# lzc452/SSL-VIT-VIDEO-ANALYTICS

Hardware: AMD Instinct MI355X
Metric: clips/sec (8x3x224x224) MAE ViT-Tiny pretrain, 1/2/4/8 GPU + recon-loss parity (higher is better)
Workload: dtype bf16; 1 GPU; BASELINE config 2: TinyViT-21M-variant MAE (stem+stages 1-3) + 4x384 decoder, T=8, 224x224, mask 0.75, bf16 autocast; model=tiny_vit_21m_variant + TinyVideoMAE, global_batch=256, per_gpu_batch=256, frames=8, image_size=224, parallelism=dp1

## Files before the change

include/sm_api.h:

```cpp
#ifndef SM_API_H
#define SM_API_H
#include <stdint.h>
#include <hip/hip_runtime_api.h>

#ifdef __cplusplus
extern "C" {
#endif

int64_t sm_gemm_workspace_bytes(int ab_dtype, int M, int N, int K);
int sm_gemm(int ab_dtype, int c_dtype, int a_layout, int b_layout, int M, int N, int K,
            const void* A, int64_t lda, const void* B, int64_t ldb, void* C, int64_t ldc,
            const float* bias, float alpha, float beta, int epi, void* aux, const void* R,
            float drop_p, uint64_t seed, const float* row_scale, int64_t rows_per_group,
            void* workspace, int64_t ws_bytes, hipStream_t stream);
int sm_gemm_persistent(int mode);
int sm_gemm_tuning(int key, int set, int value, int* prev);
int64_t sm_linear_dw_bias_workspace_bytes(int rows, int nout, int nin);
int sm_linear_dw_bias(int rows, int nout, int nin, const void* dy, const void* x, float* dW, float* db,
                      int accumulate, void* ws, int64_t ws_bytes, hipStream_t stream);
int sm_linear_dx_gelu(int M, int N, int K, const void* dy, const void* w, const void* pre, void* dx, void* h,
                      float drop_p, uint64_t seed, hipStream_t stream);
int sm_linear_dw_bias_gelu(int rows, int nout, int nin, const void* dy, const void* pre, float drop_p,
                           uint64_t seed, float* dW, float* db, int accumulate, void* ws, int64_t ws_bytes,
                           hipStream_t stream);
// ... 137 lines not shown
int64_t sm_se_workspace_bytes(int F, int HW, int C);
int sm_se_fwd(int dtype, const void* x, const float* act_mean, const float* act_rstd, const float* act_w,
              const float* act_b, int act_gelu, int F, int HW, int C, int R, const float* w1, const float* w2,
              float* pooled, float* z1, float* s, void* y, void* ws, int64_t ws_bytes, hipStream_t st);
int sm_se_bwd(int dtype, const void* dy, const void* x, const float* act_mean, const float* act_rstd,
              const float* act_w, const float* act_b, int act_gelu, int F, int HW, int C, int R,
              const float* w1, const float* w2, const float* s, const float* z1, float* dz2, float* dz1,
              void* dx, void* ws, int64_t ws_bytes, hipStream_t st);
int sm_se_scale(int dtype, const void* x, const float* act_mean, const float* act_rstd, const float* act_w,
                const float* act_b, int act_gelu, const float* s, void* y, int F, int HW, int C, hipStream_t st);
int64_t sm_se_bn_bwd_workspace_bytes(int F, int HW, int C);
int sm_se_bn_bwd(int dtype, const void* dy, const void* x, const float* bn_mean, const float* bn_rstd,
                 const float* bn_w, const float* bn_b, int bn_gelu, int F, int HW, int C, int R, const float* w1,
                 const float* w2, const float* s, const float* z1, float* dz2, float* dz1, void* dx, float* dw,
                 float* db, void* ws, int64_t ws_bytes, hipStream_t st);

int sm_tube_mask(const float* noise, int B, int T, int L, int n_mask, uint8_t* mask, int32_t* idx,
                 hipStream_t st);
int sm_pos_blend_fwd(int y_dtype, int x_dtype, const void* y, const float* tpos, const float* spos,
                     const float* tok, const uint8_t* mask, void* x, int B, int T, int L, int D,
                     hipStream_t st);
int sm_pos_blend_bwd(int g_dtype, int y_dtype, const void* dx, const uint8_t* mask, void* dy,
                     float* dtpos, float* dspos, float* dtok, float* ws, int B, int T, int L, int D,
                     hipStream_t st);
int64_t sm_loss_workspace_bytes(int B, int T, int L);
int sm_mae_loss_fwd(int pred_dtype, const void* pred, const float* clip, int64_t sB, int64_t sC,
                    int64_t sT, int64_t sH, int64_t sW, const uint8_t* mask, int B, int T, int H, int W,
                    int norm_pix, float* loss, float* denom, void* ws, int64_t ws_bytes, hipStream_t st);
int sm_mae_loss_bwd(int pred_dtype, const void* pred, const float* clip, int64_t sB, int64_t sC,
                    int64_t sT, int64_t sH, int64_t sW, const uint8_t* mask, int B, int T, int H, int W,
// ... 58 lines not shown
```

ssl-vit-video-analytics_amd/csrc/common.h:

```cpp
#pragma once
#include <hip/hip_runtime.h>
#include <stdint.h>

#define SM_DEV __device__ __forceinline__

typedef __attribute__((ext_vector_type(8))) __bf16 bf16x8;
typedef __attribute__((ext_vector_type(4))) __bf16 bf16x4;
typedef __attribute__((ext_vector_type(16))) float f32x16;
typedef __attribute__((ext_vector_type(4))) float f32x4;
typedef __attribute__((ext_vector_type(4))) short s16x4;

enum SmDtype { SM_F32 = 0, SM_BF16 = 1 };

template <typename T> SM_DEV float to_f(T x);
template <> SM_DEV float to_f<float>(float x) { return x; }
template <> SM_DEV float to_f<__bf16>(__bf16 x) { return (float)x; }
template <typename T> SM_DEV T from_f(float x);
template <> SM_DEV float from_f<float>(float x) { return x; }
template <> SM_DEV __bf16 from_f<__bf16>(float x) { return (__bf16)x; }

SM_DEV void load8(const float* p, float* v) {
  float4 a = *(const float4*)p, b = *(const float4*)(p + 4);
  v[0] = a.x; v[1] = a.y; v[2] = a.z; v[3] = a.w; v[4] = b.x; v[5] = b.y; v[6] = b.z; v[7] = b.w;
}
// ... 216 lines not shown
  __syncthreads();
  if (g == 0 && c < ncols) {
    double t = 0.0;
#pragma unroll
    for (int k = 0; k < 8; ++k) t += red[k][cl];
    if (outd) outd[c] = t;
    if (outf) outf[c] = accumulate ? outf[c] + (float)t : (float)t;
  }
}

static inline void colred(const float* part, int nb, int ncols, double* outd, float* outf, int accumulate, hipStream_t st) {
  hipLaunchKernelGGL(colred_kernel, dim3((ncols + 31) / 32), dim3(256), 0, st, part, nb, ncols, outd, outf,
                     accumulate);
}

#define SM_CHECK_LAUNCH() \
  do { hipError_t e__ = hipGetLastError(); if (e__ != hipSuccess) return (int)e__; } while (0)
```

ssl-vit-video-analytics_amd/csrc/conv.hip:

```cpp
#include <algorithm>

#include "common.h"
#include "sm_api.h"

namespace {

inline int ew_blocks(int64_t n) {
  int64_t b = (n + 255) / 256;
  if (b > 16384) b = 16384;
  return b < 1 ? 1 : (int)b;
}

struct ClipView {
  const float* p;
  int B, T, H, W;
  int64_t sB, sC, sT, sH, sW;
};

template <typename TO>
__global__ void stem_im2col_kernel(ClipView v, int Ho, int Wo, int stride, TO* col ) {
  const int64_t P = (int64_t)v.B * v.T * Ho * Wo;
  for (int64_t i = blockIdx.x * (int64_t)blockDim.x + threadIdx.x; i < P; i += (int64_t)gridDim.x * blockDim.x) {
    const int xo = (int)(i % Wo);
    const int64_t r = i / Wo;
// ... 2010 lines not shown
  double* sums = (double*)(((uintptr_t)(coef + 2 * C) + 7) & ~(uintptr_t)7);
  ChanAffine act{bn_mean, bn_rstd, bn_w, bn_b, bn_gelu};
  DISPATCH1(dtype, hipLaunchKernelGGL(se_bn_reduce_kernel<T>, dim3(ns, F), dim3(256), 0, st, (const T*)dy,
                                      (const T*)x, act, HW, C, part, part2));
  hipLaunchKernelGGL(se_fc_bwd_kernel, dim3(F), dim3(256), (C + R) * 4, st, part, ns, s, z1, w1, w2, C, R, dz2, dz1,
                     dpool);
  hipLaunchKernelGGL(se_bn_combine_kernel, dim3(F), dim3(256), 0, st, part2, ns, HW, C, s, dpool, comb);
  colred(comb, F, 2 * C, sums, nullptr, 0, st);
  hipLaunchKernelGGL(se_bn_finalize_kernel, dim3((C + 127) / 128), dim3(128), 0, st, sums, (int64_t)F * HW, C, dw,
                     db, coef);
  DISPATCH1(dtype, hipLaunchKernelGGL(se_bn_dx_kernel<T>, dim3(ns, F), dim3(256), 0, st, (const T*)dy, (const T*)x,
                                      act, s, dpool, coef, (T*)dx, HW, C));
  SM_CHECK_LAUNCH();
  return 0;
}
```

ssl-vit-video-analytics_amd/csrc/gemm.hip:

```cpp
#include "common.h"
#include "sm_api.h"
#include <stdlib.h>

namespace {

struct GemmArgs {
  int M, N, K;
  int k_begin, k_chunk;
  const void* A; int64_t lda;
  const void* B; int64_t ldb;
  void* C; int64_t ldc;
  const float* bias;
  float alpha, beta;
  int epi;
  void* aux;
  const void* R;
  float drop_p;
  uint64_t seed;
  const float* row_scale;
  int64_t rows_per_group;
  float* partial;
  float* colsum;
  int cH, cW, cC, cflip;
  float xb_p;
  uint64_t xb_seed;
  ChanAffine xb_act;
  const float* xb_gate;
  int xb_hw;
  float* stat_part;
  int ctrans;
  void* aux_out;
  const void* A2;
  int64_t lda2;
  int k1;
};

template <typename TC>
SM_DEV void epilogue_store(const GemmArgs& g, int64_t row, int col, float acc, int zs) {
  if (g.partial) {
    g.partial[(int64_t)zs * g.M * g.N + row * g.N + col] = acc;
    return;
  }
  float v = g.alpha * acc;
  if (g.bias) v += g.bias[col];
  TC* C = (TC*)g.C;
  const int64_t idx = g.ctrans ? (int64_t)col * g.ldc + row : row * g.ldc + col;
  if (g.epi & 2) v = (float)(__bf16)v;
  if (g.epi & 4) v *= gelu_grad(to_f<TC>(((const TC*)g.aux)[idx]));
  if (g.epi & 1) {
// ... 1201 lines not shown
    const int wrow = (m0 + wm) >> 6;
    const int sc = n0 + wn + 8 * l;
    const auto prs = __builtin_amdgcn_make_buffer_rsrc((void*)(g.stat_part + (int64_t)wrow * 2 * g.N), (short)0,
                                                       2 * g.N * 4, 0x00020000);
    const bool ok = l < 8 && m0 + wm < g.M && sc < g.N;
    const uint32_t o = ok ? (uint32_t)sc * 4u : BUF_OOB;
    const uint32_t o2 = ok ? (uint32_t)(g.N + sc) * 4u : BUF_OOB;
    bstore128(make_uint4(__float_as_uint(st1[0]), __float_as_uint(st1[1]), __float_as_uint(st1[2]), __float_as_uint(st1[3])), prs, o);
    bstore128(make_uint4(__float_as_uint(st1[4]), __float_as_uint(st1[5]), __float_as_uint(st1[6]), __float_as_uint(st1[7])), prs, o + 16);
    bstore128(make_uint4(__float_as_uint(st2[0]), __float_as_uint(st2[1]), __float_as_uint(st2[2]), __float_as_uint(st2[3])), prs, o2);
    bstore128(make_uint4(__float_as_uint(st2[4]), __float_as_uint(st2[5]), __float_as_uint(st2[6]), __float_as_uint(st2[7])), prs, o2 + 16);
  }
  asm volatile("s_waitcnt lgkmcnt(0)" ::: "memory");
}

template <bool BK, int IMP>
__global__ __launch_bounds__(512, 4) void gemm_bf16_pp(GemmArgs g) {
  static_assert(IMP == 0 || IMP == 8 || IMP == 9 || IMP == 11 || IMP == 12 || IMP == 13,
                "persistent form: plain, statistics, GELU backward + activation, BatchNorm-input (+ statistics) "
                "or GELU + pre epilogue");
  constexpr bool STATS = IMP == 8 || IMP == 11;
  constexpr bool XA = IMP == 11 || IMP == 12;
  __shared__ float xtab[XA ? 2 * XB_MAXK : 4];
  constexpr int BMV = 256, BNV = 128, NT = 512;
  constexpr int CHA = TileLoader<BMV, NT, true>::CH, CHB = TileLoader<BNV, NT, BK>::CH;
  constexpr int KSTEPB = TileLoader<BNV, NT, BK>::KSTEP;
  __shared__ __attribute__((aligned(16))) char lds[PP_LDS];
  char* la = lds;
  char* lb = lds + BMV * BKT * 2;
  const int w = __builtin_amdgcn_readfirstlane(threadIdx.x >> 6);
  char* img = lds + w * 8192;
  const int wm = (w >> 1) * 64, wn = (w & 1) * 64;
  const int ntn = (g.N + BNV - 1) / BNV;
  const int T = ntn * ((g.M + BMV - 1) / BMV);
  const int x = blockIdx.x & 7, qstep = gridDim.x >> 3;
  const int T8 = T >> 3, R8 = T & 7;
  const int cnt = T8 + (x < R8 ? 1 : 0), tbase = x * T8 + (x < R8 ? x : R8);
  const int it = blockIdx.x >> 3;
// ... 121 lines not shown
    put(0);
    __syncthreads();
    if (nk > 1) issue(BKT);
    kstep();
    __syncthreads();
    for (int ks = 1; ks < nk; ++ks) {
      put(ks * BKT);
      __syncthreads();
      if (ks + 1 < nk) issue((ks + 1) * BKT);
      kstep();
      __syncthreads();
    }
  };
  setup(it);
  issue(0);
  ksteps();
  int cm0 = lm0, cn0 = ln0;
  for (int in = it + qstep; in < cnt; in += qstep) {
    if constexpr (IMP == 13) pp_stage_gelu_aux(g, acc, cm0, cn0, wm, wn, opaque_tid() & 63, img);
    else if constexpr (IMP == 9) pp_stage_gelu_bwd(g, acc, cm0, cn0, wm, wn, opaque_tid() & 63, img);
    else pp_stage(g, acc, cm0, cn0, wm, wn, opaque_tid() & 63, img);
    setup(in);
    issue(0);
    if constexpr (IMP == 13 || IMP == 9) {
      if (IMP == 13 || g.aux_out) pp_flush<false>(g, IMP == 13 ? g.aux : g.aux_out, cm0, cn0, wm, wn, opaque_tid() & 63, img);
      pp_stage_runs(acc, opaque_tid() & 63, img);
    }
    pp_flush<STATS>(g, g.C, cm0, cn0, wm, wn, opaque_tid() & 63, img);
    __syncthreads();
    cm0 = lm0;
    cn0 = ln0;
    ksteps();
  }
  if constexpr (IMP == 13) {
    pp_stage_gelu_aux(g, acc, cm0, cn0, wm, wn, threadIdx.x & 63, img);
    pp_flush<false>(g, g.aux, cm0, cn0, wm, wn, threadIdx.x & 63, img);
    pp_stage_runs(acc, threadIdx.x & 63, img);
  } else if constexpr (IMP == 9) {
    pp_stage_gelu_bwd(g, acc, cm0, cn0, wm, wn, threadIdx.x & 63, img);
    if (g.aux_out) pp_flush<false>(g, g.aux_out, cm0, cn0, wm, wn, threadIdx.x & 63, img);
    pp_stage_runs(acc, threadIdx.x & 63, img);
  } else {
    pp_stage(g, acc, cm0, cn0, wm, wn, threadIdx.x & 63, img);
  }
  pp_flush<STATS>(g, g.C, cm0, cn0, wm, wn, threadIdx.x & 63, img);
}

// ... 168 lines not shown
bool mf16_ok(const GemmArgs& g) { return (g.k_chunk < g.K ? g.k_chunk : g.K) >= g_tune[TUNE_MF16_MINK]; }
template <bool BK, int IMP>
bool launch_pp(const GemmArgs& g, hipStream_t st) {
  int slots = resident_blocks<gemm_bf16_pp<BK, IMP>, 512, 2>() & ~7;
  if (slots < 8) slots = 8;
  const int64_t tiles = v2_tiles(g.M, g.N, 256);
  if (tiles <= slots) return false;
  const int rounds = pp_rounds(g);
  int64_t grid = slots;
  if (rounds > 0) {
    const int64_t per = ((tiles + 7) / 8 + rounds - 1) / rounds;
    if (8 * per > grid) grid = 8 * per;
  }
  hipLaunchKernelGGL((gemm_bf16_pp<BK, IMP>), dim3((unsigned)grid), dim3(512), 0, st, g);
  return true;
}

bool dw384_ok(int M, int N) { return g_tune[TUNE_DW384] && M % DW3_BM == 0 && N % DW3_BN == 0; }
int dw384_splits(int M, int N, int s_v2) {
  if (!dw384_ok(M, N) || s_v2 <= 1) return s_v2;
  const int tiles = (M / DW3_BM) * (N / DW3_BN);
  for (int r = 2; r >= 1; --r) {
    const int sr = r * resident_blocks<gemm_dw384<false>, 512, 1>() / tiles;
    if (sr >= 2 && sr <= s_v2) return sr;
  }
  return s_v2;
}
template <bool AK, bool BK, typename TC, bool VEC>
void launch_bf16(const GemmArgs& g, int splits, hipStream_t st) {
  if constexpr (!AK && !BK && sizeof(TC) == 4 && VEC) {
// ... 179 lines not shown

extern "C" int sm_linear_dx_gelu(int M, int N, int K, const void* dy, const void* w, const void* pre, void* dx,
                                 void* h, float drop_p, uint64_t seed, hipStream_t stream) {
  if (M <= 0 || K <= 0) return 0;
  if (N <= 0 || N % 8 || K % 8 || (((uintptr_t)dy | (uintptr_t)w | (uintptr_t)pre | (uintptr_t)dx | (uintptr_t)h) & 15))
    return -2;
  GemmArgs g{};
  g.M = M; g.N = K; g.K = N; g.A = dy; g.lda = N; g.B = w; g.ldb = K; g.C = dx; g.ldc = K;
  g.alpha = 1.f; g.beta = 0.f; g.epi = 4; g.aux = const_cast<void*>(pre); g.aux_out = h;
  g.drop_p = drop_p; g.seed = seed; g.rows_per_group = 1; g.k_begin = 0; g.k_chunk = N;
  launch_dx_gelu(g, stream);
  SM_CHECK_LAUNCH();
  return 0;
}

extern "C" int sm_linear_dx2(int M, int N, int K1, int K2, const void* a1, int64_t lda1, const void* a2, int64_t lda2,
                             const void* w, const float* bias, const void* residual, void* dx, hipStream_t stream) {
  if (M <= 0 || N <= 0) return 0;
  if (K1 <= 0 || K1 % BKT || K2 <= 0 || K2 % 8 || N % 8 || lda1 < K1 || lda2 < K2 || lda1 % 8 || lda2 % 8 ||
      a1 == nullptr || a2 == nullptr || w == nullptr || dx == nullptr ||
      (((uintptr_t)a1 | (uintptr_t)a2 | (uintptr_t)w | (uintptr_t)dx | (uintptr_t)residual) & 15))
    return -2;
  GemmArgs g{};
  g.M = M; g.N = N; g.K = K1 + K2; g.A = a1; g.lda = lda1; g.B = w; g.ldb = N; g.C = dx; g.ldc = N;
  g.A2 = a2; g.lda2 = lda2; g.k1 = K1;
  g.bias = bias; g.alpha = 1.f; g.beta = residual ? 1.f : 0.f; g.R = residual;
  g.rows_per_group = 1; g.k_begin = 0; g.k_chunk = g.K;
  launch_v2<true, false, __bf16, true, 14>(g, 1, stream);
  SM_CHECK_LAUNCH();
  return 0;
// ... 247 lines not shown
```

ssl-vit-video-analytics_amd/ssl_mae_amd/_lib.py:

```python
import ctypes
import os

import torch

_HERE = os.path.dirname(os.path.abspath(__file__))
LIB_PATH = os.environ.get("SM_LIB_PATH") or os.path.join(_HERE, "libsslmae.so")

F32, BF16 = 0, 1
_DT = {torch.float32: F32, torch.bfloat16: BF16}

_c_i32 = ctypes.c_int
_c_i64 = ctypes.c_int64
_c_f32 = ctypes.c_float
_c_u64 = ctypes.c_uint64
_c_p = ctypes.c_void_p

_SIGS = {
    "sm_gemm_workspace_bytes": (_c_i64, [_c_i32, _c_i32, _c_i32, _c_i32]),
    "sm_gemm_persistent": (_c_i32, [_c_i32]),
    "sm_gemm_tuning": (_c_i32, [_c_i32, _c_i32, _c_i32, _c_p]),
    "sm_attn_tuning": (_c_i32, [_c_i32, _c_i32, _c_i32, _c_p]),
    "sm_calibrate_mfma": (_c_i32, [_c_i32, _c_i32, _c_i32, _c_p, _c_p, _c_p]),
    "sm_gemm": (_c_i32, [_c_i32, _c_i32, _c_i32, _c_i32, _c_i32, _c_i32, _c_i32, _c_p, _c_i64, _c_p, _c_i64,
                         _c_p, _c_i64, _c_p, _c_f32, _c_f32, _c_i32, _c_p, _c_p, _c_f32, _c_u64, _c_p, _c_i64,
# ... 58 lines not shown
    "sm_stem_conv2_bn_stats": (_c_i32, [_c_p] + [_c_i32] * 3 + [_c_p] * 4 + [_c_i32] + [_c_p] * 7
                               + [_c_f32, _c_f32, _c_i32, _c_p, _c_i64, _c_p]),
    "sm_conv3x3_fwd": (_c_i32, [_c_p, _c_p, _c_p] + [_c_i32] * 5 + [_c_p]),
    "sm_conv3x3_fwd_bn_stats": (_c_i32, [_c_p, _c_p, _c_p] + [_c_i32] * 5 + [_c_p] * 5
                                + [_c_f32, _c_f32, _c_i32, _c_p, _c_i64, _c_p]),
    "sm_conv3x3_dgrad": (_c_i32, [_c_p, _c_p, _c_p] + [_c_i32] * 5 + [_c_p]),
    "sm_conv3x3_wgrad_workspace_bytes": (_c_i64, [_c_i32] * 5),
    "sm_conv3x3_wgrad": (_c_i32, [_c_p, _c_p, _c_p] + [_c_i32] * 6 + [_c_p, _c_i64, _c_p]),
    "sm_conv_wunpack_add": (_c_i32, [_c_p, _c_p, _c_i32, _c_i32, _c_i32, _c_i32, _c_p]),
    "sm_se_workspace_bytes": (_c_i64, [_c_i32, _c_i32, _c_i32]),
    "sm_se_fwd": (_c_i32, [_c_i32, _c_p] + [_c_p] * 4 + [_c_i32] * 5 + [_c_p] * 7 + [_c_i64, _c_p]),
    "sm_se_bwd": (_c_i32, [_c_i32, _c_p, _c_p] + [_c_p] * 4 + [_c_i32] * 5 + [_c_p] * 8 + [_c_i64, _c_p]),
    "sm_se_scale": (_c_i32, [_c_i32, _c_p] + [_c_p] * 4 + [_c_i32, _c_p, _c_p, _c_i32, _c_i32, _c_i32, _c_p]),
    "sm_se_bn_bwd_workspace_bytes": (_c_i64, [_c_i32, _c_i32, _c_i32]),
    "sm_se_bn_bwd": (_c_i32, [_c_i32, _c_p, _c_p] + [_c_p] * 4 + [_c_i32] * 5 + [_c_p] * 9 + [_c_p, _c_i64, _c_p]),
    "sm_dwconv_fused_partial_rows": (_c_i64, [_c_i32, _c_i32, _c_i32]),
    "sm_dwconv_fused_fwd": (_c_i32, [_c_i32] * 5 + [_c_p] * 5 + [_c_i32] + [_c_p] * 4),
    "sm_dwconv_fused_bwd_workspace_bytes": (_c_i64, [_c_i32] * 5),
    "sm_dwconv_fused_bwd": (_c_i32, [_c_i32] * 5 + [_c_p] * 6 + [_c_i32] + [_c_p] * 4 + [_c_i64, _c_p]),
    "sm_dwconv_bn_bwd_workspace_bytes": (_c_i64, [_c_i32] * 4),
    "sm_dwconv_bn_bwd": (_c_i32, [_c_i32] * 5 + [_c_p] * 6 + [_c_i32] + [_c_p] * 6 + [_c_i64, _c_p]),
    "sm_dwconv_bn_bwd_dz": (_c_i32, [_c_i32] * 5 + [_c_p] * 6 + [_c_i32] + [_c_p] * 7 + [_c_i64, _c_p]),
    "sm_linear_dx2": (_c_i32, [_c_i32] * 4 + [_c_p, _c_i64, _c_p, _c_i64] + [_c_p] * 5),
    "sm_mbconv_fold_prep": (_c_i32, [_c_i32, _c_i32] + [_c_p] * 13),
    "sm_mbconv_fold_dw": (_c_i32, [_c_i32, _c_i32, _c_i64] + [_c_p] * 11),
    "sm_bn_eval_params": (_c_i32, [_c_p, _c_p, _c_i32, _c_f32, _c_p, _c_p, _c_p]),
    "sm_segment_mean": (_c_i32, [_c_i32, _c_p, _c_i32, _c_i32, _c_i32, _c_p, _c_p]),
    "sm_segment_mean_bwd": (_c_i32, [_c_i32, _c_p, _c_i32, _c_i32, _c_i32, _c_p, _c_p]),
    "sm_bn_partials_workspace_bytes": (_c_i64, [_c_i32]),
    "sm_bn_stats_from_partials": (_c_i32, [_c_p, _c_i64, _c_i32, _c_i64] + [_c_p] * 5 + [_c_f32, _c_f32, _c_i32,
# ... 99 lines not shown
```

ssl-vit-video-analytics_amd/ssl_mae_amd/functions.py:

```python
import math

import torch

from . import ops as K

BN0_FOLD = True


class Mode:
    __slots__ = ("bf16", "act", "seed_base")

    def __init__(self, bf16, seed_base=0):
        self.bf16 = bool(bf16)
        self.act = torch.bfloat16 if bf16 else torch.float32
        self.seed_base = int(seed_base)

    def seed(self, module_index, site):
        return splitmix64(self.seed_base ^ splitmix64((module_index << 8) | site))


_M64 = (1 << 64) - 1


def splitmix64(x):
# ... 218 lines not shown
        da3 = K.bn_bwd(dout2d, a3, m5, r5, g5.detach(), b5.detach(), False, G(g5), G(b5),
                       row_scale=st.dp_scale, rows_per_group=Ho * Wo)
        if ctx.fused:
            act2 = (m2, r2, g2.detach(), b2.detach(), True)
            if (Ho * Wo) % 64 == 0:
                K.linear_dw_se(da3, a2.view(-1, mid), act2, gate, Ho * Wo, G(w_proj).view(Cout, mid))
            else:
                h3 = K.se_scale(a2, gate, Fr, Ho * Wo, mid, act=act2)
                K.linear_dw(da3, h3, G(w_proj).view(Cout, mid))
                del h3
        else:
            h2 = K.bn_apply(a2, m2, r2, g2.detach(), b2.detach(), gelu=True)
            h3 = K.se_scale(h2, gate, Fr, Ho * Wo, mid)
            K.linear_dw(da3, h3, G(w_proj).view(Cout, mid))
            del h3
        dh3 = K.linear_dx(da3, W(w_proj, mode).view(Cout, mid))
        del da3
        if ctx.fused:
            da2, dz2, dz1 = K.se_bn_bwd(dh3, a2, Fr, Ho * Wo, mid, w_fc0.detach(), w_fc2.detach(), gate, h1se,
                                        act2, G(g2), G(b2))
        else:
            dh2, dz2, dz1 = K.se_bwd(dh3, h2, Fr, Ho * Wo, mid, w_fc0.detach(), w_fc2.detach(), gate, h1se)
            del h2
            da2 = K.bn_bwd(dh2, a2, m2, r2, g2.detach(), b2.detach(), True, G(g2), G(b2))
            del dh2
        del dh3
        R = mid // 4
        K.gemm(dz2, h1se, G(w_fc2), mid, R, Fr, 1, 1, mid, R, R, beta=1.0)
        K.gemm(dz1, pooled, G(w_fc0), R, mid, Fr, 1, 1, R, mid, mid, beta=1.0)
        if a1 is None:
            a1 = expand(x)
        x2d = x.reshape(-1, Cin)
        if ctx.fused and BN0_FOLD and mid % 64 == 0 and Cin % 8 == 0 and Cin <= mid // 2:
            act0 = (m0, r0, g0.detach(), b0.detach(), True)
            dz, coef = K.dwconv_bn_bwd_dz(da2, a1, act0, w_dw.detach().view(mid, 9), G(w_dw).view(mid, 9), G(g0),
                                          G(b0), Fr, H, Wd, mid, stride=s)
# ... 213 lines not shown
```

ssl-vit-video-analytics_amd/ssl_mae_amd/kernels.py:

```python
import math

import torch

from . import _lib
from ._lib import call, dt, ptr, query, stream


def _chk(*ts):
    for t in ts:
        if t is not None and not t.is_cuda:
            raise _lib.KernelError("ssl_mae_amd kernels need device tensors (no CPU fallback)")


def _ws(nbytes, device):
    return torch.empty(max(int(nbytes), 16), dtype=torch.uint8, device=device)


def gemm(A, B, C, M, N, K, a_layout, b_layout, lda, ldb, ldc, bias=None, alpha=1.0, beta=0.0,
         gelu=False, aux=None, R=None, round_branch=False, drop_p=0.0, seed=0, row_scale=None, rows_per_group=1,
         gelu_bwd=False):
    _chk(A, B, C)
    ab = dt(A)
    if dt(B) != ab:
        raise _lib.KernelError("GEMM operands must share a dtype")
# ... 675 lines not shown

def se_bn_bwd(dy, x, F, HW, C, w1, w2, s, h1, act, dw_sink, db_sink):
    _chk(dy, x)
    R = w1.shape[0]
    dev = x.device
    dz2 = torch.empty((F, C), dtype=torch.float32, device=dev)
    dz1 = torch.empty((F, R), dtype=torch.float32, device=dev)
    dx = torch.empty_like(x)
    nbytes = query("sm_se_bn_bwd_workspace_bytes", F, HW, C)
    ws = _ws(nbytes, dev)
    call("sm_se_bn_bwd", dt(x), ptr(dy), ptr(x), *_act_args(act), F, HW, C, R, ptr(w1), ptr(w2), ptr(s), ptr(h1),
         ptr(dz2), ptr(dz1), ptr(dx), ptr(dw_sink), ptr(db_sink), ptr(ws), nbytes, stream())
    return dx, dz2, dz1


def tube_mask(noise, T, n_mask, with_index=True):
    _chk(noise)
    B, L = noise.shape
    mask = torch.empty((B, T, L), dtype=torch.uint8, device=noise.device)
    idx = torch.empty((B * T * n_mask,), dtype=torch.int32, device=noise.device) if with_index else None
    call("sm_tube_mask", ptr(noise), B, T, L, n_mask, ptr(mask), ptr(idx), stream())
    return mask, idx


def pos_blend(y, tpos, spos, tok, mask_u8, B, T, L, D, out_dtype):
    x = torch.empty((B * T * L, D), dtype=out_dtype, device=y.device)
    call("sm_pos_blend_fwd", dt(y), dt(x), ptr(y), ptr(tpos), ptr(spos), ptr(tok), ptr(mask_u8), ptr(x), B, T, L, D,
         stream())
    return x

# ... 300 lines not shown
```

ssl-vit-video-analytics_amd/ssl_mae_amd/ops.py:

```python
import torch

from . import kernels as _K

_M64 = (1 << 64) - 1


def _s64(seed):
    u = int(seed) & _M64
    return u - (1 << 64) if u >= (1 << 63) else u


def _u64(s):
    return int(s) & _M64


def _op(name, schema, mutates=()):
    def deco(impl):
        return torch.library.custom_op(f"ssl_mae::{name}", impl, mutates_args=tuple(mutates), schema=schema)
    return deco


def _none(*a, **k):
    return None

# ... 957 lines not shown
                  "Tensor(b!) db_sink) -> (Tensor, Tensor, Tensor)", ("dw_sink", "db_sink"))
def _se_bn_bwd(dy, x, F, HW, C, w1, w2, s, h1, am, ar, aw, ab, ag, dw_sink, db_sink):
    return _K.se_bn_bwd(dy, x, F, HW, C, w1, w2, s, h1, (am, ar, aw, ab, ag), dw_sink, db_sink)


@_se_bn_bwd.register_fake
def _(dy, x, F, HW, C, w1, w2, *a):
    R = w1.shape[0]
    return torch.empty_like(x), x.new_empty((F, C), dtype=torch.float32), x.new_empty((F, R), dtype=torch.float32)


def se_bn_bwd(dy, x, F, HW, C, w1, w2, s, h1, act, dw_sink, db_sink):
    return torch.ops.ssl_mae.se_bn_bwd(dy, x, F, HW, C, w1, w2, s, h1, *_act(act), dw_sink, db_sink)


@_op("tube_mask", "(Tensor noise, int T, int n_mask) -> (Tensor, Tensor)")
def _tube_mask(noise, T, n_mask):
    return _K.tube_mask(noise, T, n_mask)


@_tube_mask.register_fake
def _(noise, T, n_mask):
    B, L = noise.shape
    return noise.new_empty((B, T, L), dtype=torch.uint8), noise.new_empty(B * T * n_mask, dtype=torch.int32)


def tube_mask(noise, T, n_mask, with_index=True):
    return torch.ops.ssl_mae.tube_mask(noise, T, n_mask)


# ... 346 lines not shown
```

Before: 207.1 clips/s.

## Fuse projection dx GEMM into SE/BN2 backward reductions and dx epilogue

In the MBConv-style block backward pass, the projection linear_dx GEMM and the separate SE+BN backward are replaced by two persistent GEMM passes with custom epilogues. The first pass recomputes dh3 and reduces the per-channel SE/BN statistics directly from the accumulator. The second pass recomputes the GEMM and applies the full GELU/BN/SE backward to write dx. This avoids materialising dh3 and the extra read passes over it, at the cost of computing the small-K GEMM twice and adding register pressure in the epilogue.

```diff
diff --git a/include/sm_api.h b/include/sm_api.h
--- a/include/sm_api.h
+++ b/include/sm_api.h
@@ -175,6 +175,11 @@
                  const float* bn_w, const float* bn_b, int bn_gelu, int F, int HW, int C, int R, const float* w1,
                  const float* w2, const float* s, const float* z1, float* dz2, float* dz1, void* dx, float* dw,
                  float* db, void* ws, int64_t ws_bytes, hipStream_t st);
+int64_t sm_se_bn_bwd_proj_workspace_bytes(int F, int HW, int C);
+int sm_se_bn_bwd_proj(int dtype, const void* da3, const void* wproj, const void* x, const float* bn_mean,
+                      const float* bn_rstd, const float* bn_w, const float* bn_b, int bn_gelu, int F, int HW, int C,
+                      int Cout, int R, const float* w1, const float* w2, const float* s, const float* z1, float* dz2,
+                      float* dz1, void* dx, float* dw, float* db, void* ws, int64_t ws_bytes, hipStream_t st);
 
 int sm_tube_mask(const float* noise, int B, int T, int L, int n_mask, uint8_t* mask, int32_t* idx,
                  hipStream_t st);
diff --git a/ssl-vit-video-analytics_amd/csrc/common.h b/ssl-vit-video-analytics_amd/csrc/common.h
--- a/ssl-vit-video-analytics_amd/csrc/common.h
+++ b/ssl-vit-video-analytics_amd/csrc/common.h
@@ -254,5 +254,9 @@
                      accumulate);
 }
 
+int gemm_se_bn_proj(int pass, int M, int C, int Cout, const void* da3, const void* wproj, const void* a2,
+                    ChanAffine act, int HW, const float* s, const float* dpool, const float* coef, float* part,
+                    float* part2, void* da2, hipStream_t st);
+
 #define SM_CHECK_LAUNCH() \
   do { hipError_t e__ = hipGetLastError(); if (e__ != hipSuccess) return (int)e__; } while (0)
diff --git a/ssl-vit-video-analytics_amd/csrc/conv.hip b/ssl-vit-video-analytics_amd/csrc/conv.hip
--- a/ssl-vit-video-analytics_amd/csrc/conv.hip
+++ b/ssl-vit-video-analytics_amd/csrc/conv.hip
@@ -2048,3 +2048,39 @@
   SM_CHECK_LAUNCH();
   return 0;
 }
+
+static int se_proj_splits(int HW) { return HW / 256; }
+extern "C" int64_t sm_se_bn_bwd_proj_workspace_bytes(int F, int HW, int C) {
+  const int64_t ns = se_proj_splits(HW);
+  return (F * ns * C + (int64_t)F * C + F * ns * 4 * C + (int64_t)F * 2 * C + 2 * C) * 4 + 2 * C * 8 + 64;
+}
+
+extern "C" int sm_se_bn_bwd_proj(int dtype, const void* da3, const void* wproj, const void* x, const float* bn_mean,
+                                 const float* bn_rstd, const float* bn_w, const float* bn_b, int bn_gelu, int F,
+                                 int HW, int C, int Cout, int R, const float* w1, const float* w2, const float* s,
+                                 const float* z1, float* dz2, float* dz1, void* dx, float* dw, float* db, void* ws,
+                                 int64_t ws_bytes, hipStream_t st) {
+  if (dtype != SM_BF16 || C <= 0 || C % 8 || Cout <= 0 || Cout % 8 || Cout > 128 || F <= 0 || HW <= 0 || HW % 256 ||
+      (int64_t)F * HW > 0x7FFFFFFF || !bn_mean || !bn_gelu ||
+      (((uintptr_t)da3 | (uintptr_t)wproj | (uintptr_t)x | (uintptr_t)dx) & 15))
+    return -2;
+  if (ws_bytes < sm_se_bn_bwd_proj_workspace_bytes(F, HW, C)) return -4;
+  const int ns = se_proj_splits(HW), M = F * HW;
+  float* part = (float*)ws;
+  float* dpool = part + (int64_t)F * ns * C;
+  float* part2 = dpool + (int64_t)F * C;
+  float* comb = part2 + (int64_t)F * ns * 4 * C;
+  float* coef = comb + (int64_t)F * 2 * C;
+  double* sums = (double*)(((uintptr_t)(coef + 2 * C) + 7) & ~(uintptr_t)7);
+  ChanAffine act{bn_mean, bn_rstd, bn_w, bn_b, bn_gelu};
+  int rc = gemm_se_bn_proj(0, M, C, Cout, da3, wproj, x, act, HW, s, nullptr, nullptr, part, part2, nullptr, st);
+  if (rc) return rc;
+  hipLaunchKernelGGL(se_fc_bwd_kernel, dim3(F), dim3(256), (C + R) * 4, st, part, ns, s, z1, w1, w2, C, R, dz2, dz1,
+                     dpool);
+  hipLaunchKernelGGL(se_bn_combine_kernel, dim3(F), dim3(256), 0, st, part2, ns, HW, C, s, dpool, comb);
+  colred(comb, F, 2 * C, sums, nullptr, 0, st);
+  hipLaunchKernelGGL(se_bn_finalize_kernel, dim3((C + 127) / 128), dim3(128), 0, st, sums, (int64_t)F * HW, C, dw,
+                     db, coef);
+  SM_CHECK_LAUNCH();
+  return gemm_se_bn_proj(1, M, C, Cout, da3, wproj, x, act, HW, s, dpool, coef, nullptr, nullptr, dx, st);
+}
diff --git a/ssl-vit-video-analytics_amd/csrc/gemm.hip b/ssl-vit-video-analytics_amd/csrc/gemm.hip
--- a/ssl-vit-video-analytics_amd/csrc/gemm.hip
+++ b/ssl-vit-video-analytics_amd/csrc/gemm.hip
@@ -33,6 +33,10 @@
   const void* A2;
   int64_t lda2;
   int k1;
+  const float* se_dpool;
+  const float* se_coef;
+  float* se_part;
+  float* se_part2;
 };
 
 template <typename TC>
@@ -1264,14 +1268,189 @@
   asm volatile("s_waitcnt lgkmcnt(0)" ::: "memory");
 }
 
+constexpr int SE_TN = 128;
+SM_DEV f32x2 bf16pair(uint32_t w) { return f32x2{__uint_as_float(w << 16), __uint_as_float(w & 0xFFFF0000u)}; }
+
+SM_DEV __attribute__((always_inline)) void se_stage(const f32x16 (&acc)[2][2], int l, char* img) {
+  const int h = l >> 5;
+#pragma unroll
+  for (int i = 0; i < 2; ++i) {
+    const RowStage rs_{img + i * 4096};
+#pragma unroll
+    for (int j = 0; j < 2; ++j)
+#pragma unroll
+      for (int p = 0; p < 2; ++p) {
+        float v[8];
+#pragma unroll
+        for (int e = 0; e < 4; ++e) {
+          const auto sw = __builtin_amdgcn_permlane32_swap(__float_as_uint(acc[i][j][8 * p + e]),
+                                                           __float_as_uint(acc[i][j][8 * p + 4 + e]), false, false);
+          v[e] = __uint_as_float(sw[0]);
+          v[4 + e] = __uint_as_float(sw[1]);
+        }
+        stage_put<__bf16>(rs_, 0, j, p, h, l, v);
+      }
+  }
+}
+
+SM_DEV __attribute__((always_inline)) void se_load_a2(const GemmArgs& g, int m0, int n0, int wm, int wn, int l, int i,
+                                                      u32x4 (&av)[8]) {
+  const int colq = n0 + wn + 8 * (l & 7);
+  {
+    const int r0 = m0 + wm + 32 * i;
+    const auto prs = rows_rsrc((const __bf16*)g.aux + (int64_t)r0 * g.ldc, (int64_t)g.M - r0, g.ldc * 2);
+#pragma unroll
+    for (int q = 0; q < 4; ++q) {
+      const int r = (l >> 3) + 8 * q;
+      av[4 * i + q] = __builtin_bit_cast(u32x4, __builtin_amdgcn_raw_buffer_load_b128(
+                                                    prs, colq < g.N ? (uint32_t)((r * g.ldc + colq) * 2) : BUF_OOB, 0, 2));
+    }
+  }
+}
+
+template <int IMP>
+SM_DEV void se_tab_build(const GemmArgs& g, int m0, int n0, float* tab) {
+  const int t = opaque_tid();
+  if (t < SE_TN) {
+    const int c = n0 + t;
+    float k[6] = {0.f, 0.f, 0.f, 0.f, 0.f, 0.f};
+    if (c < g.N) {
+      const float rs = g.xb_act.rstd[c], mu = g.xb_act.mean[c], w = g.xb_act.w[c];
+      k[0] = rs * w;
+      k[1] = bn_shift(g.xb_act.b[c], mu, k[0]);
+      if constexpr (IMP == 15) {
+        k[2] = rs;
+        k[3] = mu * rs;
+      } else {
+        const int64_t fc = (int64_t)(m0 / g.xb_hw) * g.N + c;
+        const float wr = w * rs, k1 = g.se_coef[g.N + c], inv = 1.f / (float)g.xb_hw;
+        k[2] = wr * g.xb_gate[fc];
+        k[3] = wr * (g.se_dpool[fc] * inv);
+        k[4] = wr * (k1 * (mu * rs) - g.se_coef[c]);
+        k[5] = wr * k1 * rs;
+      }
+    }
+#pragma unroll
+    for (int e = 0; e < (IMP == 15 ? 4 : 6); ++e) tab[e * SE_TN + t] = k[e];
+  }
+}
+
+SM_DEV __attribute__((always_inline)) void se_reduce_epi(const GemmArgs& g, const u32x4 (&av)[8], int w, int l,
+                                                         const char* img, const float* tab, float* red) {
+  asm volatile("s_waitcnt lgkmcnt(0)" ::: "memory");
+  const int c = l & 7;
+  typedef __attribute__((ext_vector_type(2))) __bf16 bf16x2;
+#pragma unroll
+  for (int jp = 0; jp < 4; ++jp) {
+    const int tc = (w & 1) * 64 + 8 * c + 2 * jp;
+    const f32x2 sc = *(const f32x2*)(tab + tc), sh = *(const f32x2*)(tab + SE_TN + tc);
+    const f32x2 rs = *(const f32x2*)(tab + 2 * SE_TN + tc), mr = *(const f32x2*)(tab + 3 * SE_TN + tc);
+    f32x2 acc[5];
+#pragma unroll
+    for (int s = 0; s < 5; ++s) acc[s] = f32x2{0.f, 0.f};
+#pragma unroll
+    for (int i = 0; i < 2; ++i)
+#pragma unroll
+      for (int q = 0; q < 4; ++q) {
+        const int r = (l >> 3) + 8 * q;
+        const f32x2 gy = bf16pair(*(const uint32_t*)(img + i * 4096 + r * 128 + ((c ^ rs_swz(r)) << 4) + 4 * jp));
+        const f32x2 v = bf16pair(av[4 * i + q][jp]);
+        const f32x2 u = vfma(v, sc, sh);
+        f32x2 pdf;
+        const f32x2 cdf = gelu_phi_pair_t<f32x2>(u, &pdf);
+        f32x2 hv;
+        {
+#pragma clang fp contract(off)
+          hv = u * cdf;
+        }
+        const f32x2 gp = vfma(u, pdf, cdf);
+        const f32x2 xh = vfma(v, rs, -mr);
+        const bf16x2 hb = {(__bf16)hv[0], (__bf16)hv[1]};
+        const f32x2 hh = bf16pair(__builtin_bit_cast(uint32_t, hb));
+        const f32x2 t = gp * xh;
+        acc[0] = vfma(gy, hh, acc[0]);
+        acc[1] = vfma(gy, gp, acc[1]);
+        acc[2] += gp;
+        acc[3] = vfma(gy, t, acc[3]);
+        acc[4] += t;
+        if (q & 1) __builtin_amdgcn_sched_barrier(0);
+      }
+#pragma unroll
+    for (int s = 0; s < 5; ++s) {
+      const float s0 = xor8_16_32_sum(acc[s][0]), s1 = xor8_16_32_sum(acc[s][1]);
+      if (l < 8) *(f32x2*)(red + (w * 5 + s) * 64 + 8 * c + 2 * jp) = f32x2{s0, s1};
+    }
+  }
+}
+
+SM_DEV __attribute__((always_inline)) void se_part_store(const GemmArgs& g, int m0, int n0, const float* red) {
+  const int t = opaque_tid();
+  const int cl = t & (SE_TN - 1), h = cl >> 6, cc = cl & 63;
+  const int64_t tm = m0 >> 8;
+  const bool ok = t < SE_TN && n0 + cl < g.N;
+  const auto r1 = __builtin_amdgcn_make_buffer_rsrc((void*)(g.se_part + tm * g.N), (short)0, g.N * 4, 0x00020000);
+  const auto r2 = __builtin_amdgcn_make_buffer_rsrc((void*)(g.se_part2 + tm * 4 * g.N), (short)0, 4 * g.N * 4, 0x00020000);
+#pragma unroll
+  for (int s = 0; s < 5; ++s) {
+    const float* p = red + s * 64 + cc;
+    const float a = ((p[h * 320] + p[(2 + h) * 320]) + p[(4 + h) * 320]) + p[(6 + h) * 320];
+    const uint32_t o = ok ? (uint32_t)((s ? (s - 1) * g.N : 0) + n0 + cl) * 4u : BUF_OOB;
+    __builtin_amdgcn_raw_buffer_store_b32(__float_as_uint(a), s ? r2 : r1, o, 0, 0);
+  }
+}
+
+SM_DEV __attribute__((always_inline)) void se_dx_epi(const GemmArgs& g, u32x4 (&av)[8], int m0, int n0, int wm, int wn,
+                                                     int l, const char* img, const float* tab) {
+  asm volatile("s_waitcnt lgkmcnt(0)" ::: "memory");
+  const int c = l & 7;
+  const int col = n0 + wn + 8 * c;
+  const bool cok = col < g.N;
+#pragma unroll
+  for (int i = 0; i < 2; ++i) {
+    u32x4 dv[4];
+#pragma unroll
+    for (int q = 0; q < 4; ++q) {
+      const int r = (l >> 3) + 8 * q;
+      dv[q] = *(const u32x4*)(img + i * 4096 + r * 128 + ((c ^ rs_swz(r)) << 4));
+    }
+#pragma unroll
+    for (int jp = 0; jp < 4; ++jp) {
+      const int tc = wn + 8 * c + 2 * jp;
+      const f32x2 sc = *(const f32x2*)(tab + tc), sh = *(const f32x2*)(tab + SE_TN + tc);
+      const f32x2 ka = *(const f32x2*)(tab + 2 * SE_TN + tc), kb = *(const f32x2*)(tab + 3 * SE_TN + tc);
+      const f32x2 c0 = *(const f32x2*)(tab + 4 * SE_TN + tc), c1 = *(const f32x2*)(tab + 5 * SE_TN + tc);
+#pragma unroll
+      for (int q = 0; q < 4; ++q) {
+        const f32x2 v = bf16pair(av[4 * i + q][jp]), gy = bf16pair(dv[q][jp]);
+        const f32x2 gd = gelu_grad2(vfma(v, sc, sh));
+        const f32x2 of = vfma(gd, vfma(gy, ka, kb), vfma(-c1, v, c0));
+        typedef __attribute__((ext_vector_type(2))) __bf16 bf16x2;
+        const bf16x2 o = {(__bf16)of[0], (__bf16)of[1]};
+        av[4 * i + q][jp] = __builtin_bit_cast(uint32_t, o);
+        if (q & 1) __builtin_amdgcn_sched_barrier(0);
+      }
+    }
+    const int r0 = m0 + wm + 32 * i;
+    const auto rs = rows_rsrc((const __bf16*)g.C + (int64_t)r0 * g.ldc, (int64_t)g.M - r0, g.ldc * 2);
+#pragma unroll
+    for (int q = 0; q < 4; ++q) {
+      const int r = (l >> 3) + 8 * q;
+      __builtin_amdgcn_raw_buffer_store_b128(av[4 * i + q], rs, cok ? (uint32_t)((r * g.ldc + col) * 2) : BUF_OOB, 0, 2);
+    }
+  }
+  asm volatile("s_waitcnt lgkmcnt(0)" ::: "memory");
+}
+
 template <bool BK, int IMP>
 __global__ __launch_bounds__(512, 4) void gemm_bf16_pp(GemmArgs g) {
-  static_assert(IMP == 0 || IMP == 8 || IMP == 9 || IMP == 11 || IMP == 12 || IMP == 13,
-                "persistent form: plain, statistics, GELU backward + activation, BatchNorm-input (+ statistics) "
-                "or GELU + pre epilogue");
+  static_assert(IMP == 0 || IMP == 8 || IMP == 9 || IMP == 11 || IMP == 12 || IMP == 13 || IMP == 15 || IMP == 16,
+                "persistent form: plain, statistics, GELU backward + activation, BatchNorm-input (+ statistics), "
+                "GELU + pre or SE / BN2 backward (reduce, dx) epilogue");
   constexpr bool STATS = IMP == 8 || IMP == 11;
   constexpr bool XA = IMP == 11 || IMP == 12;
-  __shared__ float xtab[XA ? 2 * XB_MAXK : 4];
+  constexpr bool SE = IMP == 15 || IMP == 16;
+  __shared__ __attribute__((aligned(16))) float xtab[XA ? 2 * XB_MAXK : SE ? 6 * SE_TN : 4];
+  __shared__ __attribute__((aligned(16))) float sered[IMP == 15 ? 8 * 5 * 64 : 4];
   constexpr int BMV = 256, BNV = 128, NT = 512;
   constexpr int CHA = TileLoader<BMV, NT, true>::CH, CHB = TileLoader<BNV, NT, BK>::CH;
   constexpr int KSTEPB = TileLoader<BNV, NT, BK>::KSTEP;
@@ -1423,9 +1602,27 @@
   };
   setup(it);
   issue(0);
+  if constexpr (SE) se_tab_build<IMP>(g, lm0, ln0, xtab);
   ksteps();
   int cm0 = lm0, cn0 = ln0;
   for (int in = it + qstep; in < cnt; in += qstep) {
+    if constexpr (SE) {
+      u32x4 av[8];
+      se_stage(acc, opaque_tid() & 63, img);
+      se_load_a2(g, cm0, cn0, wm, wn, opaque_tid() & 63, 0, av);
+      se_load_a2(g, cm0, cn0, wm, wn, opaque_tid() & 63, 1, av);
+      if constexpr (IMP == 15) se_reduce_epi(g, av, w, opaque_tid() & 63, img, xtab, sered);
+      else se_dx_epi(g, av, cm0, cn0, wm, wn, opaque_tid() & 63, img, xtab);
+      setup(in);
+      issue(0);
+      __syncthreads();
+      se_tab_build<IMP>(g, lm0, ln0, xtab);
+      if constexpr (IMP == 15) se_part_store(g, cm0, cn0, sered);
+      cm0 = lm0;
+      cn0 = ln0;
+      ksteps();
+      continue;
+    }
     if constexpr (IMP == 13) pp_stage_gelu_aux(g, acc, cm0, cn0, wm, wn, opaque_tid() & 63, img);
     else if constexpr (IMP == 9) pp_stage_gelu_bwd(g, acc, cm0, cn0, wm, wn, opaque_tid() & 63, img);
     else pp_stage(g, acc, cm0, cn0, wm, wn, opaque_tid() & 63, img);
@@ -1440,6 +1637,20 @@
     cm0 = lm0;
     cn0 = ln0;
     ksteps();
+  }
+  if constexpr (SE) {
+    u32x4 av[8];
+    se_stage(acc, threadIdx.x & 63, img);
+    se_load_a2(g, cm0, cn0, wm, wn, threadIdx.x & 63, 0, av);
+    se_load_a2(g, cm0, cn0, wm, wn, threadIdx.x & 63, 1, av);
+    if constexpr (IMP == 15) {
+      se_reduce_epi(g, av, w, threadIdx.x & 63, img, xtab, sered);
+      __syncthreads();
+      se_part_store(g, cm0, cn0, sered);
+    } else {
+      se_dx_epi(g, av, cm0, cn0, wm, wn, threadIdx.x & 63, img, xtab);
+    }
+    return;
   }
   if constexpr (IMP == 13) {
     pp_stage_gelu_aux(g, acc, cm0, cn0, wm, wn, threadIdx.x & 63, img);
@@ -1638,6 +1849,12 @@
   }
   hipLaunchKernelGGL((gemm_bf16_pp<BK, IMP>), dim3((unsigned)grid), dim3(512), 0, st, g);
   return true;
+}
+template <bool BK, int IMP>
+void launch_pp_any(const GemmArgs& g, hipStream_t st) {
+  if (launch_pp<BK, IMP>(g, st)) return;
+  const int64_t grid = 8 * ((v2_tiles(g.M, g.N, 256) + 7) / 8);
+  hipLaunchKernelGGL((gemm_bf16_pp<BK, IMP>), dim3((unsigned)grid), dim3(512), 0, st, g);
 }
 
 bool dw384_ok(int M, int N) { return g_tune[TUNE_DW384] && M % DW3_BM == 0 && N % DW3_BN == 0; }
@@ -1847,6 +2064,23 @@
   return 0;
 }
 
+int gemm_se_bn_proj(int pass, int M, int C, int Cout, const void* da3, const void* wproj, const void* a2,
+                    ChanAffine act, int HW, const float* s, const float* dpool, const float* coef, float* part,
+                    float* part2, void* da2, hipStream_t st) {
+  if (M <= 0 || HW <= 0 || HW % 256 || M % HW || C <= 0 || C % 8 || Cout <= 0 || Cout % 8 || Cout > 2 * BKT ||
+      (((uintptr_t)da3 | (uintptr_t)wproj | (uintptr_t)a2 | (uintptr_t)da2) & 15))
+    return -2;
+  GemmArgs g{};
+  g.M = M; g.N = C; g.K = Cout; g.A = da3; g.lda = Cout; g.B = wproj; g.ldb = C; g.C = da2; g.ldc = C;
+  g.alpha = 1.f; g.beta = 0.f; g.rows_per_group = 1; g.k_begin = 0; g.k_chunk = Cout;
+  g.aux = const_cast<void*>(a2); g.xb_act = act; g.xb_hw = HW; g.xb_gate = s;
+  g.se_dpool = dpool; g.se_coef = coef; g.se_part = part; g.se_part2 = part2;
+  if (pass == 0) launch_pp_any<false, 15>(g, st);
+  else launch_pp_any<false, 16>(g, st);
+  SM_CHECK_LAUNCH();
+  return 0;
+}
+
 extern "C" int sm_linear_dx2(int M, int N, int K1, int K2, const void* a1, int64_t lda1, const void* a2, int64_t lda2,
                              const void* w, const float* bias, const void* residual, void* dx, hipStream_t stream) {
   if (M <= 0 || N <= 0) return 0;
diff --git a/ssl-vit-video-analytics_amd/ssl_mae_amd/_lib.py b/ssl-vit-video-analytics_amd/ssl_mae_amd/_lib.py
--- a/ssl-vit-video-analytics_amd/ssl_mae_amd/_lib.py
+++ b/ssl-vit-video-analytics_amd/ssl_mae_amd/_lib.py
@@ -96,6 +96,9 @@
     "sm_se_scale": (_c_i32, [_c_i32, _c_p] + [_c_p] * 4 + [_c_i32, _c_p, _c_p, _c_i32, _c_i32, _c_i32, _c_p]),
     "sm_se_bn_bwd_workspace_bytes": (_c_i64, [_c_i32, _c_i32, _c_i32]),
     "sm_se_bn_bwd": (_c_i32, [_c_i32, _c_p, _c_p] + [_c_p] * 4 + [_c_i32] * 5 + [_c_p] * 9 + [_c_p, _c_i64, _c_p]),
+    "sm_se_bn_bwd_proj_workspace_bytes": (_c_i64, [_c_i32, _c_i32, _c_i32]),
+    "sm_se_bn_bwd_proj": (_c_i32, [_c_i32, _c_p, _c_p, _c_p] + [_c_p] * 4 + [_c_i32] * 6 + [_c_p] * 9
+                          + [_c_p, _c_i64, _c_p]),
     "sm_dwconv_fused_partial_rows": (_c_i64, [_c_i32, _c_i32, _c_i32]),
     "sm_dwconv_fused_fwd": (_c_i32, [_c_i32] * 5 + [_c_p] * 5 + [_c_i32] + [_c_p] * 4),
     "sm_dwconv_fused_bwd_workspace_bytes": (_c_i64, [_c_i32] * 5),
diff --git a/ssl-vit-video-analytics_amd/ssl_mae_amd/functions.py b/ssl-vit-video-analytics_amd/ssl_mae_amd/functions.py
--- a/ssl-vit-video-analytics_amd/ssl_mae_amd/functions.py
+++ b/ssl-vit-video-analytics_amd/ssl_mae_amd/functions.py
@@ -5,6 +5,7 @@
 from . import ops as K
 
 BN0_FOLD = True
+SE_PROJ_FUSE = True
 
 
 class Mode:
@@ -256,12 +257,19 @@
             h3 = K.se_scale(h2, gate, Fr, Ho * Wo, mid)
             K.linear_dw(da3, h3, G(w_proj).view(Cout, mid))
             del h3
-        dh3 = K.linear_dx(da3, W(w_proj, mode).view(Cout, mid))
-        del da3
-        if ctx.fused:
+        wp = W(w_proj, mode).view(Cout, mid)
+        proj_fused = SE_PROJ_FUSE and ctx.fused and mode.bf16 and K.se_bn_bwd_proj_ok(da3, wp, a2, Ho * Wo)
+        dh3 = None if proj_fused else K.linear_dx(da3, wp)
+        if proj_fused:
+            da2, dz2, dz1 = K.se_bn_bwd_proj(da3, wp, a2, Fr, Ho * Wo, mid, w_fc0.detach(), w_fc2.detach(), gate,
+                                             h1se, act2, G(g2), G(b2))
+            del da3
+        elif ctx.fused:
+            del da3
             da2, dz2, dz1 = K.se_bn_bwd(dh3, a2, Fr, Ho * Wo, mid, w_fc0.detach(), w_fc2.detach(), gate, h1se,
                                         act2, G(g2), G(b2))
         else:
+            del da3
             dh2, dz2, dz1 = K.se_bwd(dh3, h2, Fr, Ho * Wo, mid, w_fc0.detach(), w_fc2.detach(), gate, h1se)
             del h2
             da2 = K.bn_bwd(dh2, a2, m2, r2, g2.detach(), b2.detach(), True, G(g2), G(b2))
diff --git a/ssl-vit-video-analytics_amd/ssl_mae_amd/kernels.py b/ssl-vit-video-analytics_amd/ssl_mae_amd/kernels.py
--- a/ssl-vit-video-analytics_amd/ssl_mae_amd/kernels.py
+++ b/ssl-vit-video-analytics_amd/ssl_mae_amd/kernels.py
@@ -713,6 +713,27 @@
     return dx, dz2, dz1
 
 
+def se_bn_bwd_proj_ok(da3, wproj, x, HW):
+    Cout, C = wproj.shape
+    return (da3.dtype == wproj.dtype == x.dtype == torch.bfloat16 and C % 8 == 0 and Cout % 8 == 0 and Cout <= 128
+            and HW % 256 == 0)
+
+
+def se_bn_bwd_proj(da3, wproj, x, F, HW, C, w1, w2, s, h1, act, dw_sink, db_sink):
+    _chk(da3, wproj, x)
+    R = w1.shape[0]
+    Cout = wproj.shape[0]
+    dev = x.device
+    dz2 = torch.empty((F, C), dtype=torch.float32, device=dev)
+    dz1 = torch.empty((F, R), dtype=torch.float32, device=dev)
+    dx = torch.empty_like(x)
+    nbytes = query("sm_se_bn_bwd_proj_workspace_bytes", F, HW, C)
+    ws = _ws(nbytes, dev)
+    call("sm_se_bn_bwd_proj", dt(x), ptr(da3), ptr(wproj), ptr(x), *_act_args(act), F, HW, C, Cout, R, ptr(w1),
+         ptr(w2), ptr(s), ptr(h1), ptr(dz2), ptr(dz1), ptr(dx), ptr(dw_sink), ptr(db_sink), ptr(ws), nbytes, stream())
+    return dx, dz2, dz1
+
+
 def tube_mask(noise, T, n_mask, with_index=True):
     _chk(noise)
     B, L = noise.shape
diff --git a/ssl-vit-video-analytics_amd/ssl_mae_amd/ops.py b/ssl-vit-video-analytics_amd/ssl_mae_amd/ops.py
--- a/ssl-vit-video-analytics_amd/ssl_mae_amd/ops.py
+++ b/ssl-vit-video-analytics_amd/ssl_mae_amd/ops.py
@@ -995,6 +995,26 @@
     return torch.ops.ssl_mae.se_bn_bwd(dy, x, F, HW, C, w1, w2, s, h1, *_act(act), dw_sink, db_sink)
 
 
+@_op("se_bn_bwd_proj", "(Tensor da3, Tensor wproj, Tensor x, int F, int HW, int C, Tensor w1, Tensor w2, Tensor s, "
+                       "Tensor h1, Tensor act_mean, Tensor act_rstd, Tensor act_w, Tensor act_b, bool act_gelu, "
+                       "Tensor(a!) dw_sink, Tensor(b!) db_sink) -> (Tensor, Tensor, Tensor)", ("dw_sink", "db_sink"))
+def _se_bn_bwd_proj(da3, wproj, x, F, HW, C, w1, w2, s, h1, am, ar, aw, ab, ag, dw_sink, db_sink):
+    return _K.se_bn_bwd_proj(da3, wproj, x, F, HW, C, w1, w2, s, h1, (am, ar, aw, ab, ag), dw_sink, db_sink)
+
+
+@_se_bn_bwd_proj.register_fake
+def _(da3, wproj, x, F, HW, C, w1, w2, *a):
+    R = w1.shape[0]
+    return torch.empty_like(x), x.new_empty((F, C), dtype=torch.float32), x.new_empty((F, R), dtype=torch.float32)
+
+
+se_bn_bwd_proj_ok = _K.se_bn_bwd_proj_ok
+
+
+def se_bn_bwd_proj(da3, wproj, x, F, HW, C, w1, w2, s, h1, act, dw_sink, db_sink):
+    return torch.ops.ssl_mae.se_bn_bwd_proj(da3, wproj, x, F, HW, C, w1, w2, s, h1, *_act(act), dw_sink, db_sink)
+
+
 @_op("tube_mask", "(Tensor noise, int T, int n_mask) -> (Tensor, Tensor)")
 def _tube_mask(noise, T, n_mask):
     return _K.tube_mask(noise, T, n_mask)
```

After: 208.6 clips/s (median of 6 runs). About the same (+0.7%).
